# Kuuro-neko/HAI719-Raytracing

Measured on AMD Instinct MI355X. Metric: Msamples/s (pixels x spp / s), Cornell+mesh 1080p@256spp, higher is better.
Workload: dtype f32

## Files before the change

hai719-raytracing_amd/csrc/hrt_api.hip:

```cpp
#include "hrt_kernels.hip"
#include "hrt_dual.hip"
#include "hrt_stream.hip"
#include "hrt_output.hip"
#include "hrt_kat.hip"
#include "hrt_pack.h"

#include <dlfcn.h>
#include <rccl/rccl.h>

#include <array>
#include <cfloat>
#include <chrono>
#include <cmath>
#include <cstdio>
#include <cstdlib>
#include <cstddef>
#include <cstring>
#include <new>
#include <string>
#include <thread>
#include <unordered_map>
#include <vector>

namespace {
// ... 449 lines not shown
}

static int fill_render(hrt_scene *s, const hrt_camera *cam, uint32_t w, uint32_t h, uint32_t spp, uint64_t seed,
                       uint32_t flags, uint32_t rank, uint32_t world, DRender &R, DCamera &C) {
    const int frc = check_frame("render", w, h, k_max_pixels);
    if (frc != HRT_OK) return frc;
    if (!spp) return fail(HRT_ERR_INVALID, "render: spp must be positive");
    if (w > 65535u || h > 65535u) return fail(HRT_ERR_INVALID, "render: w and h must be below 65536 (tile origins are packed in 16 + 16 bits)");
    if (!world || rank >= world) return fail(HRT_ERR_INVALID, "render: bad rank/world");
    R.scene = s->d_scene;
    R.lds_units = (flags & HRT_FLAG_NO_LDS_TREE) ? 0u : s->lds_units;
    R.err_abs = margin_scale(s->bound, std::sqrt(cam->eye[0] * cam->eye[0] + cam->eye[1] * cam->eye[1] + cam->eye[2] * cam->eye[2]));
    {
        const int crc = make_camera(cam, C);
        if (crc != HRT_OK) return crc;
    }
    R.w = w; R.h = h; R.spp = spp;
    R.seed_lo = (uint32_t)seed; R.seed_hi = (uint32_t)(seed >> 32);
    R.flags = flags;
    R.rank = rank; R.world = world;
    R.tiles_x = (w + HRT_TILE - 1) / HRT_TILE;
    R.tiles_total = hrt_tiles_total(w, h);
    R.tiles_owned = hrt_tiles_owned(w, h, rank, world);
    R.tile_counter = s->tile_counter;
    R.stamps = s->stamps;
    R.tile_list = nullptr;
    return HRT_OK;
}

static int size_stream(hrt_scene *s, const KernelBuild &b, DRender &R, uint32_t &grid, uint32_t &lds_bytes) {
    const uint32_t fixed = (uint32_t)(HRT_SP_NQ * HRT_SP_POOL * 2 + HRT_SP_STREAMS * sizeof(SpCtl) + sizeof(SpShared) + HRT_SP_UNITS * sizeof(SpUnit) + HRT_SP_UNITS * HRT_SP_MAXG * 4) +
                           ((b.bits & KB_VIEWS) ? HRT_SP_UNITS * HRT_SP_MAXG * 16u : 0u) +
                           2048u + s->d.tab_rows * 16u
#ifdef HRT_WALK_SEG
                           + 2048u
#endif
                           ;
    uint32_t per_cu = (64u * 4u * HRT_SP_MINW) / HRT_SP_WG;
    while (per_cu > 1u && 160u * 1024u / per_cu < fixed + 16u * 1024u) --per_cu;
    const uint32_t room = (160u * 1024u / per_cu - fixed) / 16u;
    if (!(R.flags & HRT_FLAG_NO_LDS_TREE)) R.lds_units = std::min<uint32_t>(s->d.n_kd_units, room) & ~3u;
    lds_bytes = fixed + R.lds_units * 16u;
    grid = std::min<uint32_t>((uint32_t)g_rt.cus * per_cu, R.tiles_owned);
    {
        const uint32_t per_tile = 64u * std::min<uint32_t>(R.spp, HRT_SP_SCHUNK);
        uint32_t glog = 0;
        while ((2u << glog) <= HRT_SP_MAXG && (per_tile << (glog + 1u)) <= HRT_SP_UNIT) ++glog;
        R.sp_group_log2 = glog;
        uint32_t band = 0;
        while (glog == 0u && band < 2u && ((uint64_t)R.tiles_owned << band) < 64ull * grid && (64u >> (band + 1u)) * (uint64_t)std::min<uint32_t>(R.spp, HRT_SP_SCHUNK) >= 4096u) ++band;
        R.sp_band_log2 = band;
    }
    int rc = s->sp_scratch.grow((size_t)grid * HRT_SP_UNITS * HRT_SP_UNIT * 3u * sizeof(float));
    if (rc == HRT_OK) rc = s->sp_pool.grow((size_t)grid * SP_FIELDS * HRT_SP_POOL * sizeof(uint32_t));
    if (rc != HRT_OK) return rc;
    R.sp_scratch = s->sp_scratch.as<float>();
    R.sp_pool = s->sp_pool.as<uint32_t>();
    return HRT_OK;
}

static int size_lanes(const KernelBuild &b, DRender &R, uint32_t &grid, uint32_t &lds_bytes) {
    const bool dual = b.family == KF_DUAL;
    lds_bytes = R.lds_units * 16u;
    if (dual) {
        const uint32_t wgs = 1024u / HRT_WG, backup = HRT_DS_FIELDS * HRT_WG * 4u;
        const uint32_t room = (156u * 1024u / wgs - backup) / 16u;
        if (R.lds_units > room) R.lds_units = room & ~3u;
        lds_bytes = R.lds_units * 16u + backup;
    }
    int per_cu = 0;
    HIP_TRY(hipOccupancyMaxActiveBlocksPerMultiprocessor(&per_cu, (const void *)b.fn, HRT_WG, lds_bytes));
    if (per_cu < 1) per_cu = 1;
    grid = (uint32_t)(per_cu * g_rt.cus);
    const uint32_t per_wg = (HRT_WG / 64u) * (dual ? 2u : 1u);
    const uint32_t need = (R.tiles_owned + per_wg - 1u) / per_wg;
    if (grid > need) grid = need;
    R.sp_scratch = nullptr;
    R.sp_pool = nullptr;
    return HRT_OK;
}

struct TraceJob {
    uint32_t w, h, s0, spp;
    uint64_t seed;
    uint32_t flags;
    float *d_tiles;
    void *stream;
    uint32_t rank = 0, world = 1;
    bool accumulate = false;
    const uint32_t *list = nullptr;
    uint32_t list_n = 0;
    uint32_t n_views = 0;
};
static int launch_trace(hrt_scene *s, const hrt_camera *cam, const TraceJob &J) {
    DRender R;
    DCamera C;
    int rc = fill_render(s, cam, J.w, J.h, J.spp, J.seed, J.flags, J.rank, J.world, R, C);
    if (rc != HRT_OK) return rc;
    if (J.list) {
        if (J.list_n > R.tiles_owned) return fail(HRT_ERR_INVALID, "render: tile list longer than the rank's tiles");
        R.tile_list = J.list;
        R.tiles_owned = J.list_n;
    }
    if (J.n_views) {
        R.views = s->vw_blocks.as<DView>();
        R.tiles_owned = J.n_views * R.tiles_total;
    }
// ... 378 lines not shown
```

hai719-raytracing_amd/csrc/hrt_stream.hip:

```cpp
#include "hrt_device.h"

#ifndef HRT_SP_POOL
#define HRT_SP_POOL 4096
#endif
#ifndef HRT_SP_WG
#define HRT_SP_WG 1024
#endif
#ifndef HRT_SP_MINW
#define HRT_SP_MINW 4
#endif
#define HRT_SP_SCHUNK 1024
#ifndef HRT_SP_UNIT
#define HRT_SP_UNIT 8192
#endif
#ifndef HRT_SP_UNITS
#define HRT_SP_UNITS 4
#endif
#define HRT_SP_MAXG 16
#ifndef HRT_SP_TRIPS
#define HRT_SP_TRIPS 6
#endif
#ifndef HRT_SP_TPRIO
#define HRT_SP_TPRIO 3
#endif
#ifndef HRT_SP_VOTE
#define HRT_SP_VOTE 0
#endif
#ifndef HRT_SP_STEPS
#define HRT_SP_STEPS 16
#endif
#ifndef HRT_SP_CYCLE_BOUND
#define HRT_SP_CYCLE_BOUND (1u << 16)
#endif
#ifndef HRT_SP_WAIT_SECONDS
#define HRT_SP_WAIT_SECONDS 900ull
#endif
#ifndef HRT_SP_GIVEUP_AFTER
#define HRT_SP_GIVEUP_AFTER 0u
#endif
#ifndef HRT_SP_STREAMS
#define HRT_SP_STREAMS 2
#endif
#ifndef HRT_SP_PMQ
#define HRT_SP_PMQ 1
#endif
#ifndef HRT_SP_THALF
#define HRT_SP_THALF 0
#endif
#ifndef HRT_SP_DEFER
#define HRT_SP_DEFER 1
#endif
#ifndef HRT_SP_PRUNE
#define HRT_SP_PRUNE 3
#endif
#define HRT_SP_QCAP (HRT_SP_POOL / HRT_SP_STREAMS)
#define HRT_SP_NQ 8

namespace hrtk {

enum { SP_OX = 0, SP_OY, SP_OZ, SP_DX, SP_DY, SP_DZ, SP_HT, SP_HID,
       SP_TR, SP_TG, SP_TB, SP_RR, SP_RG, SP_RB, SP_RI, SP_REM,
       SP_WTRI, SP_WTE, SP_WKK, SP_WBT, SP_WREF, SP_WBU, SP_WBV, SP_PM,
       SP_FREE = 24,
       SP_FIELDS = 32 };

struct SpCtl {
    uint32_t cQ[6][2];
    uint32_t cursor;
    uint32_t ngen, gen_n0;
    uint32_t gen_slot, gen_s0;
    uint32_t red_slot;
    uint32_t red_j, red_s0, red_ns;
    uint32_t more;
    uint32_t done, parity;
    uint32_t arrive;
    uint32_t ready;
    uint32_t pad[2];
};
struct SpUnit {
    uint32_t state;
    uint32_t j;
    uint32_t s0, ns;
    uint32_t gen_next, gen_total;
    uint32_t outstanding;
    uint32_t pad;
};
enum { SP_U_FREE = 0, SP_U_READY, SP_U_GENERATING, SP_U_DRAINING, SP_U_REDUCING };
struct SpShared {
    uint32_t lock;
    uint32_t cur;
    uint32_t tiles_done;
    uint32_t abort;
    uint32_t stall;
    uint32_t sections;
    uint32_t pad[2];
};
static_assert(sizeof(SpCtl) % 16 == 0 && sizeof(SpShared) % 16 == 0 && sizeof(SpUnit) % 16 == 0, "the LDS regions behind the control blocks must stay 16-byte aligned");
static_assert(HRT_SP_STREAMS == 1 || HRT_SP_STREAMS == 2, "one or two streams");
static_assert(HRT_SP_UNITS >= 1 && HRT_SP_UNITS <= 4, "a path number carries its unit slot in its two top bits");
static_assert(!HRT_SP_PMQ || HRT_SP_POOL <= 4096, "a T-queue entry is 12 bits of slot id + 4 bits of meshes");
static_assert(HRT_SP_UNIT <= 8192, "g3.w keeps 13 bits of the path's number in its unit beside the bounces left");
static_assert(HRT_SP_QCAP >= 512, "deferring partial chunks needs a queue that can hold a whole chunk whenever fewer than 64 slots are free (6 queues x 63 < QCAP - 64)");

static_assert((HRT_SP_POOL & (HRT_SP_POOL - 1)) == 0 && HRT_SP_POOL <= 65536, "slot ids are 16-bit and masked with HRT_SP_POOL - 1");
static_assert(HRT_SP_NQ * HRT_SP_POOL * 2 + HRT_SP_MAXG * 8 + 512 <= 160 * 1024, "the queues do not fit the CU's 160 KB of LDS");

struct SpLds {
    uint32_t *st;
    uint16_t *q;
    SpCtl *ctl;
};

#define SP_AT(field, slot) ((slot) * (uint32_t)SP_FIELDS + (uint32_t)(field))
__device__ __forceinline__ uint4 sp_ld4(const SpLds &L, int g, uint32_t slot) {
    const v4u v = ((gu4)(L.st + SP_AT(4 * g, slot)))[0];
    return make_uint4(v.x, v.y, v.z, v.w);
}
__device__ __forceinline__ void sp_st4(const SpLds &L, int g, uint32_t slot, uint4 v) {
    v4u w;
    w.x = v.x; w.y = v.y; w.z = v.z; w.w = v.w;
    *((v4u __attribute__((address_space(1))) *)(L.st + SP_AT(4 * g, slot))) = w;
}
#define SP_PIN1(g) "+v"(g.x), "+v"(g.y), "+v"(g.z), "+v"(g.w)
__device__ __forceinline__ uint32_t sp_w7(uint32_t left, uint32_t pnum) { return left | ((pnum & 0x1FFFu) << 3) | (pnum & 0xC0000000u); }
__device__ __forceinline__ uint32_t sp_w7_left(uint32_t w) { return w & 7u; }
__device__ __forceinline__ uint32_t sp_w7_pnum(uint32_t w) { return ((w >> 3) & 0x1FFFu) | (w & 0xC0000000u); }
static_assert(HRT_MAX_SOUP_SLOTS == (1u << 25), "the hit word keeps 25 bits of soup slot");
__device__ __forceinline__ uint32_t sp_hit_word(const Hit &h) {
    return h.kind == 3u ? (3u << 30) | (h.index << 25) | h.tri : (h.kind << 30) | h.index;
}
__device__ __forceinline__ void sp_hit_unword(uint32_t w, Hit &h) {
    h.kind = w >> 30;
    const bool mesh = h.kind == 3u;
    h.index = mesh ? (w >> 25) & 31u : w & 0x3FFFFFFFu;
    h.tri = mesh ? w & 0x01FFFFFFu : 0u;
}
__device__ __forceinline__ uint4 sp_pack(float a, float b, float c, float d) { return make_uint4(__float_as_uint(a), __float_as_uint(b), __float_as_uint(c), __float_as_uint(d)); }
__device__ __forceinline__ void sp_unpack_ray_hit(const uint4 g0, const uint4 g1, Ray &ray, Hit &h) {
    ray.o = mk(__uint_as_float(g0.x), __uint_as_float(g0.y), __uint_as_float(g0.z));
    ray.d = mk(__uint_as_float(g0.w), __uint_as_float(g1.x), __uint_as_float(g1.y));
    h.t = __uint_as_float(g1.z);
    sp_hit_unword(g1.w, h);
    h.a0 = 0.f; h.a1 = 0.f;
}
__device__ __forceinline__ uint4 sp_g1(const Ray &ray, const Hit &h) {
    return make_uint4(__float_as_uint(ray.d.y), __float_as_uint(ray.d.z), __float_as_uint(h.t), sp_hit_word(h));
}
__device__ __forceinline__ void sp_store_ray_hit(const SpLds &L, uint32_t slot, const Ray &ray, const Hit &h) {
    sp_st4(L, 0, slot, sp_pack(ray.o.x, ray.o.y, ray.o.z, ray.d.x));
    sp_st4(L, 1, slot, sp_g1(ray, h));
}
template <class CX>
__device__ __forceinline__ void sp_hit_uv_square(const CX &cx, const Ray &ray, Hit &h) {
    float t, u = 0.f, v = 0.f;
    if (quad_t(cx.tq + HRT_QUAD_ROWS * h.index, ray, HRT_FLT_MAX, t, u, v)) { h.a0 = u; h.a1 = v; }
}
template <class CX>
__device__ __forceinline__ void sp_hit_uv_triangle(const CX &cx, const Ray &ray, Hit &h) {
    const gf4 tr = (gf4)cx.S->tris + HRT_TRI_ROWS * h.tri;
    float u1, u2;
    (void)tri_inside(ld(tr, 0), ld(tr, 1), ld(tr, 2), ray, h.t, u1, u2);
    h.a0 = u1; h.a1 = u2;
}
__device__ __forceinline__ uint16_t *spq(const SpLds &L, int which, uint32_t parity) { return L.q + (2 * which + parity) * HRT_SP_QCAP; }

#define SP_TO_NONE 6u
__device__ __forceinline__ void sp_push_all(const SpLds &L, SpCtl &C, uint32_t out, uint32_t to, uint32_t slot) {
    uint32_t rank = 0, count = 0, leader = 0;
#pragma unroll
    for (uint32_t q = 0; q < 6u; ++q) {
        const uint64_t m = __ballot(to == q);
        if (to == q) {
            rank = __builtin_amdgcn_mbcnt_hi((uint32_t)(m >> 32), __builtin_amdgcn_mbcnt_lo((uint32_t)m, 0u));
            count = (uint32_t)__popcll(m);
            leader = (uint32_t)__builtin_ctzll(m | (1ull << 63));
        }
    }
    uint32_t base = 0;
    if (to < SP_TO_NONE && rank == 0u) base = atomicAdd(&C.cQ[to][out], count);
    base = __shfl(base, (int)leader);
    if (to < SP_TO_NONE) {
        const uint32_t pos = base + rank;
        const uint32_t buf = to == 0u ? 0u : (to == 5u ? 3u : ((to == 2u || to == 3u) ? 1u : 2u));
        const bool back = to == 3u || to == 4u;
        spq(L, (int)buf, out)[back ? (uint32_t)HRT_SP_QCAP - 1u - pos : pos] = (uint16_t)slot;
    }
}

template <bool LIGHTS, bool EXACT = false, bool SPHF = false, bool LIST = false, bool VIEWS = false>
__device__ __forceinline__ void stream_body(const DRender &R) {
    extern __shared__ uint4 s_raw[];
    SpLds L;
    L.st = R.sp_pool + (size_t)blockIdx.x * ((size_t)SP_FIELDS * HRT_SP_POOL);
    L.q = reinterpret_cast<uint16_t *>(s_raw);
    L.ctl = reinterpret_cast<SpCtl *>(L.q + HRT_SP_NQ * HRT_SP_POOL);
    SpShared &SH = *reinterpret_cast<SpShared *>(L.ctl + HRT_SP_STREAMS);
    SpUnit *const U = reinterpret_cast<SpUnit *>(&SH + 1);
    uint32_t *tile_xy = reinterpret_cast<uint32_t *>(U + HRT_SP_UNITS);
    uint4 *tile_vw = reinterpret_cast<uint4 *>(tile_xy + HRT_SP_UNITS * HRT_SP_MAXG);
    float *s_lut = VIEWS ? reinterpret_cast<float *>(tile_vw + HRT_SP_UNITS * HRT_SP_MAXG)
                         : reinterpret_cast<float *>(tile_xy + HRT_SP_UNITS * HRT_SP_MAXG);
    float4 *s_tabs = reinterpret_cast<float4 *>(s_lut + 512);
    CtxT<EXACT, true, SPHF> cx;
    cx.S = (cscene)R.scene;
    const uint32_t tab_rows = cx.S->tab_rows;
    uint4 *s_units = reinterpret_cast<uint4 *>(s_tabs + tab_rows);
    cx.set_tables((lf4)s_tabs, (lf1)s_lut, cx.S);
    cx.lds = (lu4)s_units;
    cx.lds_n = R.lds_units;
    cx.err_abs = R.err_abs;
    cx.flags = R.flags;
    unsigned long long stamps_local[17];
    cx.st = stamps_local;
#ifdef HRT_WALK_SEG
    {
        unsigned long long *wseg = reinterpret_cast<unsigned long long *>(s_units + R.lds_units) + (threadIdx.x >> 6) * 16u;
        if ((threadIdx.x & 63u) < 16u) wseg[threadIdx.x & 63u] = 0ull;
        cx.st = wseg;
    }
#endif
    ccam cam = (ccam)R.cam;
    const uint32_t tid = threadIdx.x, lane = tid & 63u;
    {
        gu4 g_units = (gu4)cx.S->kd_units;
        for (uint32_t i = tid; i < cx.lds_n; i += HRT_SP_WG) s_units[i] = ld(g_units, i);
        gf4 g_tabs = (gf4)cx.S->tabs;
        for (uint32_t i = tid; i < tab_rows; i += HRT_SP_WG) s_tabs[i] = ld(g_tabs, i);
        if (tid < 512u) s_lut[tid] = c_u8_lut[tid];
    }
    uint16_t *const q_all = L.q;
    if (tid < HRT_SP_STREAMS) {
        SpCtl &C0 = L.ctl[tid];
        C0.cQ[0][0] = C0.cQ[0][1] = 0;
        for (int k = 0; k < 4; ++k) C0.cQ[1 + k][0] = C0.cQ[1 + k][1] = 0;
        C0.cQ[5][0] = HRT_SP_QCAP; C0.cQ[5][1] = 0;
        C0.parity = 1; C0.done = 0; C0.arrive = 0; C0.ready = 0; C0.cursor = 0; C0.ngen = 0; C0.gen_n0 = 0; C0.gen_slot = 0; C0.gen_s0 = 0;
        C0.red_slot = HRT_SP_UNITS; C0.red_j = 0; C0.red_s0 = 0; C0.red_ns = 0; C0.more = 1;
        if (tid == 0) {
            SH.lock = 0; SH.cur = 0; SH.tiles_done = 0; SH.abort = 0; SH.stall = 0; SH.sections = 0;
            for (int k = 0; k < HRT_SP_UNITS; ++k) { U[k].state = SP_U_FREE; U[k].j = 0; U[k].s0 = 0; U[k].ns = 0; U[k].gen_next = 0; U[k].gen_total = 0; U[k].outstanding = 0; }
        }
    }
    for (uint32_t i = tid; i < HRT_SP_POOL; i += HRT_SP_WG)
        q_all[(i / HRT_SP_QCAP) * (HRT_SP_NQ * HRT_SP_QCAP) + (2 * 3 + 0) * HRT_SP_QCAP + (i % HRT_SP_QCAP)] = (uint16_t)i;
    const bool has_mesh = cx.S->n_meshes != 0u;
    const bool multi_mesh = cx.S->n_meshes > 1u;
#if HRT_SP_PMQ
    const bool pm_in_entry = cx.S->n_meshes <= 4u;
#endif
    const bool prune = !EXACT && HRT_SP_PRUNE != 0 && cx.S->prune_ok != 0u;
    const bool moving = cx.S->any_motion != 0u;
    const bool sky_is_zero = cx.S->skybox_image < 0 && cx.S->dark_sky != 0;
    float *scratch = R.sp_scratch + (size_t)blockIdx.x * ((size_t)HRT_SP_UNITS * HRT_SP_UNIT * 3u);
    const uint32_t glog = R.sp_group_log2, G = 1u << glog, blog = R.sp_band_log2;
    const uint32_t upix = (64u << glog) >> blog, upix_log2 = 6u + glog - blog;
    const uint32_t items = R.tiles_owned << blog;
    auto view_row = [&](uint32_t pnum) { return tile_vw[(pnum >> 30) * HRT_SP_MAXG + (((pnum & 0x3FFFFFFFu) & (upix - 1u)) >> 6)]; };
#define SP_UNI(x) __builtin_amdgcn_readfirstlane(x)

#ifndef HRT_SP_SEG_KIND
#define HRT_SP_SEG_KIND 1
#endif
#ifdef HRT_SP_SEG
    unsigned long long seg[10] = {0, 0, 0, 0, 0, 0, 0, 0, 0, 0}, seg_last = 0;
    bool seg_on = false;
#define SEG_START(on) do { seg_on = (on); if (seg_on) { asm volatile("s_waitcnt vmcnt(0) lgkmcnt(0)" ::: "memory"); seg_last = __builtin_readcyclecounter(); } } while (0)
#define SEG(k) do { if (seg_on) { asm volatile("s_waitcnt vmcnt(0) lgkmcnt(0)" ::: "memory"); const unsigned long long t_ = __builtin_readcyclecounter(); \
                                  seg[k] += t_ - seg_last; seg_last = t_; } } while (0)
#else
#define SEG_START(on) do { } while (0)
#define SEG(k) do { } while (0)
#endif
#ifdef HRT_SP_DEBUG
    unsigned long long dbg_work = 0, dbg_chunks = 0, dbg_cycles = 0, dbg_serial = 0, dbg_wait = 0, dbg_drain = 0, dbg_tail = 0, dbg_tail_cycles = 0;
    unsigned long long dbg_class[6] = {0, 0, 0, 0, 0, 0};
    const unsigned long long dbg_t0 = __builtin_readcyclecounter();
#endif
    const uint32_t per_fold = min((uint32_t)HRT_SP_SCHUNK, (uint32_t)HRT_SP_UNIT / upix);
    auto serial_section = [&](SpCtl &C, uint16_t *qs) {
        const uint32_t par = SP_UNI(C.parity) ^ 1u;
        const uint32_t free_in = SP_UNI(C.cQ[5][par]);
#if HRT_SP_DEFER
        const uint32_t want = free_in & ~63u;
#else
        const uint32_t want = free_in;
#endif
        if (lane == 0) {
            uint32_t spins = 0;
            while (atomicCAS(&SH.lock, 0u, 1u) != 0u) {
                __builtin_amdgcn_s_sleep(1);
// ... 61 lines not shown
                    atomicAdd(&u.outstanding, ngen);
                    if (u.gen_next == u.gen_total) u.state = SP_U_DRAINING;
                    gs = cur;
                }
            }
            bool generating = false, idle = SH.tiles_done != 0u;
            for (uint32_t k = 0; k < HRT_SP_UNITS; ++k) {
                generating = generating || U[k].state == SP_U_READY || U[k].state == SP_U_GENERATING || (U[k].state == SP_U_FREE && SH.tiles_done == 0u);
                idle = idle && U[k].state == SP_U_FREE;
            }
            C.ngen = ngen; C.gen_n0 = n0; C.gen_slot = gs; C.gen_s0 = U[gs].s0;
            C.more = generating ? 1u : 0u;
            C.done = idle ? 1u : 0u;
            uint32_t entries = ngen + (red < HRT_SP_UNITS ? 1u : 0u);
            for (int q = 0; q < 5; ++q) entries += (HRT_SP_DEFER && generating) ? (C.cQ[q][par] & ~63u) : C.cQ[q][par];
            const uint32_t stalled = entries != 0u ? (SH.stall = 0u) : ++SH.stall;
            const uint32_t sections = ++SH.sections;
            if (stalled > HRT_SP_CYCLE_BOUND || (HRT_SP_GIVEUP_AFTER != 0u && sections > HRT_SP_GIVEUP_AFTER)) {
                if (R.stamps) {
                    __hip_atomic_store(R.stamps + 15, 0xDEADull, __ATOMIC_RELAXED, __HIP_MEMORY_SCOPE_SYSTEM);
                    R.stamps[14] = 2;
                    for (uint32_t k = 0; k < HRT_SP_UNITS; ++k) R.stamps[8 + k] = ((unsigned long long)U[k].state << 48) | ((unsigned long long)U[k].outstanding << 24) | U[k].gen_next;
                    R.stamps[12] = ((unsigned long long)SH.tiles_done << 32) | SH.cur; R.stamps[13] = ((unsigned long long)want << 32) | C.cQ[0][par];
                }
                __hip_atomic_store(&SH.abort, 1u, __ATOMIC_RELAXED, __HIP_MEMORY_SCOPE_WORKGROUP);
            }
            __hip_atomic_store(&SH.lock, 0u, __ATOMIC_RELEASE, __HIP_MEMORY_SCOPE_WORKGROUP);
        }
        asm volatile("s_waitcnt lgkmcnt(0)" ::: "memory");
        const uint32_t ngen = SP_UNI(C.ngen);
        uint16_t *qFi = qs + (2 * 3 + par) * HRT_SP_QCAP, *qFo = qs + (2 * 3 + (par ^ 1u)) * HRT_SP_QCAP;
        for (uint32_t i = lane; i < free_in - ngen; i += 64u) qFo[i] = qFi[ngen + i];
        const bool defer = HRT_SP_DEFER && SP_UNI(C.more) != 0u;
        const uint32_t cT = SP_UNI(C.cQ[0][par]), rT = defer ? (cT & 63u) : 0u;
        if (lane < rT) qs[(2 * 0 + (par ^ 1u)) * HRT_SP_QCAP + lane] = qs[(2 * 0 + par) * HRT_SP_QCAP + cT - rT + lane];
        uint32_t cKv[4], rK[4], waiting = cT;
#pragma unroll
        for (int k = 0; k < 4; ++k) {
            cKv[k] = SP_UNI(C.cQ[1 + k][par]);
            rK[k] = defer ? (cKv[k] & 63u) : 0u;
            waiting += cKv[k];
            const int which = (k == 1 || k == 2) ? 1 : 2;
            const bool back = !(k == 1 || k == 0);
            const uint16_t *qi = qs + (2 * which + par) * HRT_SP_QCAP;
            uint16_t *qo = qs + (2 * which + (par ^ 1u)) * HRT_SP_QCAP;
            if (lane < rK[k]) {
                const uint32_t e = cKv[k] - rK[k] + lane;
                qo[back ? (uint32_t)HRT_SP_QCAP - 1u - lane : lane] = qi[back ? (uint32_t)HRT_SP_QCAP - 1u - e : e];
            }
        }
        if (lane == 0) {
#pragma unroll
            for (int k = 0; k < 4; ++k) { C.cQ[1 + k][par] = cKv[k] - rK[k]; C.cQ[1 + k][par ^ 1u] = rK[k]; }
            C.cQ[0][par] = cT - rT;
            C.cQ[0][par ^ 1u] = rT;
            C.cQ[5][par ^ 1u] = free_in - ngen;
            C.cursor = 0; C.parity = par;
            C.done = (C.done != 0u && ngen == 0u && waiting == 0u && C.red_slot == HRT_SP_UNITS) ? 1u : 0u;
        }
        asm volatile("s_waitcnt lgkmcnt(0)" ::: "memory");
        if (lane == 0) __hip_atomic_store(&C.ready, C.ready + 1u, __ATOMIC_RELEASE, __HIP_MEMORY_SCOPE_WORKGROUP);
    };
    __syncthreads();
    if (tid < 64u)
        for (uint32_t st = 0; st < HRT_SP_STREAMS; ++st) serial_section(L.ctl[st], q_all + st * (HRT_SP_NQ * HRT_SP_QCAP));
    __syncthreads();
    uint32_t fin[HRT_SP_UNITS];
    for (int k = 0; k < HRT_SP_UNITS; ++k) fin[k] = 0u;

    uint32_t kcyc[HRT_SP_STREAMS], fin_mask = 0u;
    for (uint32_t st = 0; st < HRT_SP_STREAMS; ++st) kcyc[st] = 1u;
    for (uint32_t round = 0;; ++round) {
        const uint32_t st = HRT_SP_STREAMS == 1 ? 0u : (round & 1u);
        if (fin_mask == (1u << HRT_SP_STREAMS) - 1u) break;
        if (fin_mask & (1u << st)) continue;
        SpCtl &C = L.ctl[st];
        L.q = q_all + st * (HRT_SP_NQ * HRT_SP_QCAP);
        {
#ifdef HRT_SP_DEBUG
            const unsigned long long dbg_q0 = __builtin_readcyclecounter();
#endif
            uint32_t spins = 0, aborted = 0;
            const unsigned long long wait_t0 = __builtin_amdgcn_s_memrealtime();
            while (SP_UNI(__hip_atomic_load(&C.ready, __ATOMIC_ACQUIRE, __HIP_MEMORY_SCOPE_WORKGROUP)) < kcyc[st]) {
                __builtin_amdgcn_s_sleep(8);
                aborted = SP_UNI(__hip_atomic_load(&SH.abort, __ATOMIC_RELAXED, __HIP_MEMORY_SCOPE_WORKGROUP));
                if (aborted) break;
                if ((++spins & 1023u) == 0u && (spins >> 10) > 16u && __builtin_amdgcn_s_memrealtime() - wait_t0 > 100000000ull * HRT_SP_WAIT_SECONDS) {
                    if (lane == 0) {
                        if (R.stamps) { __hip_atomic_store(R.stamps + 15, 0xDEADull, __ATOMIC_RELAXED, __HIP_MEMORY_SCOPE_SYSTEM); R.stamps[14] = 3; }
                        __hip_atomic_store(&SH.abort, 1u, __ATOMIC_RELAXED, __HIP_MEMORY_SCOPE_WORKGROUP);
                    }
                    aborted = 1u;
                    break;
                }
            }
#ifdef HRT_SP_DEBUG
            dbg_wait += __builtin_readcyclecounter() - dbg_q0;
#endif
            if (aborted || SP_UNI(__hip_atomic_load(&SH.abort, __ATOMIC_RELAXED, __HIP_MEMORY_SCOPE_WORKGROUP))) break;
        }
        if (SP_UNI(C.done)) { fin_mask |= 1u << st; continue; }
        const uint32_t parity = SP_UNI(C.parity);
        const uint32_t ngen = SP_UNI(C.ngen), n0 = SP_UNI(C.gen_n0), gs = SP_UNI(C.gen_slot), s0 = SP_UNI(C.gen_s0);
        const uint32_t red = SP_UNI(C.red_slot), nR = red < HRT_SP_UNITS ? (upix * 3u + 63u) >> 6 : 0u;
        const uint32_t cTin = SP_UNI(C.cQ[0][parity]);
        const uint32_t cK0 = SP_UNI(C.cQ[1][parity]), cK1 = SP_UNI(C.cQ[2][parity]), cK2 = SP_UNI(C.cQ[3][parity]),
                       cK3 = SP_UNI(C.cQ[4][parity]);
        const uint32_t nT = HRT_SP_THALF ? (cTin + 31u) >> 5 : (cTin + 63u) >> 6, e3 = nT + ((cK3 + 63u) >> 6), e1 = e3 + ((cK1 + 63u) >> 6),
                       e2 = e1 + ((cK2 + 63u) >> 6), e0 = e2 + ((cK0 + 63u) >> 6), nG = (ngen + 63u) >> 6, total = e0 + nG;
        uint16_t *qTi = spq(L, 0, parity);
        uint16_t *qAi = spq(L, 1, parity), *qBi = spq(L, 2, parity);
        uint16_t *qFi = spq(L, 3, parity);
#ifdef HRT_SP_DEBUG
        const unsigned long long dbg_w0 = __builtin_readcyclecounter();
        ++dbg_cycles;
#endif

        for (;;) {
            uint32_t c = 0;
            if (lane == 0) c = atomicAdd(&C.cursor, 1u);
            c = SP_UNI(c);
            if (c >= nR + total) break;
            if (c < nR) {
                const uint32_t i = c * 64u + lane;
                const uint32_t rj = SP_UNI(C.red_j), rs0 = SP_UNI(C.red_s0), rns = SP_UNI(C.red_ns);
                if (i < upix * 3u && rj + i / (192u >> blog) < items) {
                    float *out = R.out_tiles + (size_t)rj * (192u >> blog) + i;
                    float acc = (rs0 != 0u || R.accumulate) ? *out : 0.f;
                    const float *col = scratch + (size_t)red * ((size_t)HRT_SP_UNIT * 3u) + i;
                    const uint32_t stride = upix * 3u;
                    uint32_t sm = 0;
                    for (; sm + 8u <= rns; sm += 8u) {
                        float v[8];
#pragma unroll
                        for (int k = 0; k < 8; ++k) v[k] = col[(size_t)(sm + k) * stride];
#pragma unroll
                        for (int k = 0; k < 8; ++k) acc += v[k];
                    }
                    for (; sm < rns; ++sm) acc += col[(size_t)sm * stride];
                    if (rs0 + rns >= R.spp) {
                        const uint32_t q = i / 3u, p = q & 63u, txy = tile_xy[red * HRT_SP_MAXG + (q >> 6)];
                        const uint32_t px = (txy & 0xFFFFu) + (p & 7u), py = (txy >> 16) + (p >> 3);
                        if (!(px < R.w && py < R.h)) acc = 0.f;
                        else if (!R.accumulate) acc = acc / (float)R.spp;
                    }
                    *out = acc;
                }
                continue;
            }
            c -= nR;
#ifdef HRT_SP_DEBUG
            ++dbg_chunks;
            const unsigned long long dbg_c0 = __builtin_readcyclecounter();
            const uint32_t dbg_k = c < nT ? 0u : (c < e3 ? 1u : (c < e1 ? 2u : (c < e2 ? 3u : (c < e0 ? 4u : 5u))));
#endif
            if (c < nT) {
#if HRT_SP_TPRIO
                __builtin_amdgcn_s_setprio(HRT_SP_TPRIO);
#endif
                const uint32_t e = HRT_SP_THALF ? c * 32u + lane : c * 64u + lane;
                const bool act = e < cTin && (!HRT_SP_THALF || lane < 32u);
                uint32_t slot = 0, kind = 0, pm = 0, t_before = 0;
                bool walked = false;
                Ray ray;
                ray.o = mk(0.f, 0.f, 0.f); ray.d = mk(0.f, 0.f, 1.f); ray.time = 0.f;
                Hit h;
                h.kind = 0; h.index = 0; h.t = HRT_FLT_MAX; h.tri = 0; h.a0 = 0.f; h.a1 = 0.f;
                Walk w;
                w.ref = HRT_KD_NIL; w.t_entry = 0.f; w.kk = 0xFFFFu; w.best_t = HRT_FLT_MAX; w.best_tri = 0; w.bu = 0.f; w.bv = 0.f;
                SEG_START(HRT_SP_SEG_KIND == 2);
                if (act) {
#if HRT_SP_PMQ
                    const uint32_t entry = qTi[e];
                    slot = entry & (HRT_SP_POOL - 1u);
#else
                    slot = qTi[e] & (HRT_SP_POOL - 1u);
#endif
                    uint4 g0 = sp_ld4(L, 0, slot), g1 = sp_ld4(L, 1, slot), g4 = sp_ld4(L, 4, slot), g5 = sp_ld4(L, 5, slot);
                    asm volatile("" : SP_PIN1(g0), SP_PIN1(g1), SP_PIN1(g4), SP_PIN1(g5));
                    sp_unpack_ray_hit(g0, g1, ray, h);
                    pm = g5.w;
                    t_before = g1.z;
                    w.ref = g5.x; w.t_entry = __uint_as_float(g4.y); w.kk = g4.z; w.best_t = __uint_as_float(g4.w);
                    w.best_tri = g4.x; w.bu = __uint_as_float(g5.y); w.bv = __uint_as_float(g5.z);
#if HRT_SP_PMQ
                    if (pm_in_entry && (entry >> 12) != 0u) { w.ref = HRT_KD_NIL; pm = entry >> 12; }
#endif
                }
#ifdef HRT_SP_SEG
                asm volatile("" : "+v"(ray.o.x), "+v"(w.t_entry), "+v"(h.t));
#endif
                SEG(0);
                if (act) {
#if HRT_SP_VOTE
                    walked = walk_vote(cx, ray, pm, w, h, HRT_SP_STEPS);
#else
                    walked = multi_mesh ? walk_some_per_lane(cx, ray, pm, w, h, HRT_SP_TRIPS) : walk_some(cx, ray, pm, w, h, HRT_SP_TRIPS);
#endif
                }
                SEG(1);
                if (act) {
                    if (__float_as_uint(h.t) != t_before) sp_st4(L, 1, slot, sp_g1(ray, h));
                    if (!walked) {
                        sp_st4(L, 4, slot, make_uint4(w.best_tri, __float_as_uint(w.t_entry), w.kk, __float_as_uint(w.best_t)));
                        sp_st4(L, 5, slot, make_uint4(w.ref, __float_as_uint(w.bu), __float_as_uint(w.bv), pm));
                    }
                    kind = h.kind;
                }
#if HRT_SP_TPRIO
                __builtin_amdgcn_s_setprio(0);
#endif
                sp_push_all(L, C, parity ^ 1u, !act ? SP_TO_NONE : (walked ? 1u + kind : 0u), slot);
                SEG(2);
#ifdef HRT_SP_SEG
                if (seg_on) { seg[7] += 1; seg[6] += (unsigned long long)__popcll(__ballot(act)); seg[5] += (unsigned long long)__popcll(__ballot(act && walked)); }
#endif
            } else {
                const bool is_gen = c >= e0;
                const uint32_t first = is_gen ? e0 : (c < e3 ? nT : (c < e1 ? e3 : (c < e2 ? e1 : e2)));
                const uint32_t fill = is_gen ? ngen : (c < e3 ? cK3 : (c < e1 ? cK1 : (c < e2 ? cK2 : cK0)));
                const bool from_back = !is_gen && (c < e3 || (c >= e1 && c < e2));
                const uint16_t *qHi = (c < e3 || c >= e2) ? qBi : qAi;
                const uint32_t e = (c - first) * 64u + lane;
                const bool act = e < fill;
                uint32_t slot = 0, kind = 0, fin_unit = 0, pnum = 0;
                bool trace = false, freed = false;
                bool ended = false, last_seg = false;
                f3 rad = mk(0.f, 0.f, 0.f);
                SEG_START((HRT_SP_SEG_KIND == 1 && !is_gen && c >= e1 && c < e2) || (HRT_SP_SEG_KIND == 3 && !is_gen && c >= e3 && c < e1) ||
                          (HRT_SP_SEG_KIND == 4 && is_gen) || (HRT_SP_SEG_KIND == 5 && !is_gen && c < e3));
                Ray ray;
                ray.o = mk(0.f, 0.f, 0.f); ray.d = mk(0.f, 0.f, 1.f); ray.time = 0.f;
                if (act && is_gen) {
                    slot = qFi[e] & (HRT_SP_POOL - 1u);
                    const uint32_t n = n0 + e;
                    const uint32_t q = n & (upix - 1u), s = s0 + (n >> upix_log2);
                    const uint32_t p = q & 63u, txy = tile_xy[gs * HRT_SP_MAXG + (q >> 6)];
                    const uint32_t px = (txy & 0xFFFFu) + (p & 7u), py = (txy >> 16) + (p >> 3);
                    if (txy != 0xFFFFFFFFu && px < R.w && py < R.h) {
                        uint4 vw = make_uint4(0u, R.seed_lo, R.seed_hi, 0u);
                        if (VIEWS) { vw = view_row(n | (gs << 30)); cx.err_abs = __uint_as_float(vw.w); }
                        Rng rng;
                        rng.start(vw.y, vw.z, py * R.w + px, R.s0 + s);
                        const float u = ((float)px + rng.next()) / (float)R.w;
                        const float v = ((float)py + rng.next()) / (float)R.h;
                        const float tm = rng.next();
                        if (VIEWS) {
                            for (uint64_t todo = __ballot(1); todo != 0ull;) {
                                const uint32_t view = __builtin_amdgcn_readlane(vw.x, __builtin_ctzll(todo));
                                const bool mine = vw.x == view;
                                if (mine) ray = camera_ray<EXACT>((ccam)&((cview)R.views + view)->cam, u, v, tm);
                                todo &= ~__ballot(mine);
                            }
                        } else {
                            ray = camera_ray<EXACT>(cam, u, v, tm);
                        }
                        pnum = n | (gs << 30);
                        sp_st4(L, 2, slot, sp_pack(1.f, 1.f, 1.f, 0.f));
                        sp_st4(L, 3, slot, make_uint4(0u, 0u, rng.i, sp_w7(6u, pnum)));
                        trace = true;
                    } else {
                        float *o = scratch + (size_t)gs * ((size_t)HRT_SP_UNIT * 3u) + (size_t)n * 3u;
                        o[0] = 0.f; o[1] = 0.f; o[2] = 0.f;
                        freed = true;
                        fin_unit = gs;
                    }
                } else if (act) {
                    slot = qHi[from_back ? (uint32_t)HRT_SP_QCAP - 1u - e : e] & (HRT_SP_POOL - 1u);
                    uint4 g0 = sp_ld4(L, 0, slot), g1 = sp_ld4(L, 1, slot), g2 = sp_ld4(L, 2, slot), g3 = sp_ld4(L, 3, slot);
                    asm volatile("" : SP_PIN1(g0), SP_PIN1(g1), SP_PIN1(g2), SP_PIN1(g3));
                    pnum = sp_w7_pnum(g3.w);
                    Rng key;
                    {
                        const uint32_t kn = pnum & 0x3FFFFFFFu, ku = pnum >> 30;
                        const uint32_t kq = kn & (upix - 1u), ks = U[ku].s0 + (kn >> upix_log2);
                        const uint32_t kxy = tile_xy[ku * HRT_SP_MAXG + (kq >> 6)];
                        const uint32_t kx = (kxy & 0xFFFFu) + (kq & 7u), ky = (kxy >> 16) + ((kq & 63u) >> 3);
                        uint4 vw = make_uint4(0u, R.seed_lo, R.seed_hi, 0u);
                        if (VIEWS) { vw = view_row(pnum); cx.err_abs = __uint_as_float(vw.w); }
                        key.start(vw.y, vw.z, ky * R.w + kx, R.s0 + ks);
                        key.i = 2u;
                    }
                    Hit h;
                    sp_unpack_ray_hit(g0, g1, ray, h);
                    ray.time = moving ? key.next() : 0.f;
                    f3 thr = mk(__uint_as_float(g2.x), __uint_as_float(g2.y), __uint_as_float(g2.z));
                    rad = mk(__uint_as_float(g2.w), __uint_as_float(g3.x), __uint_as_float(g3.y));
                    int remaining = (int)sp_w7_left(g3.w);
#ifdef HRT_SP_SEG
                    asm volatile("" : "+v"(remaining), "+v"(ray.o.x), "+v"(thr.x), "+v"(rad.x));
#endif
                    SEG(0);
                    if (h.kind == 0u) {
                        rad = rad + thr * sky(cx, ray.d, remaining);
                        ended = true;
                    } else {
                        Rng rng;
                        rng.k0 = key.k0; rng.k1 = key.k1; rng.i = g3.z;
                        if (h.kind == 2u) sp_hit_uv_square(cx, ray, h);
                        else if (h.kind == 3u) sp_hit_uv_triangle(cx, ray, h);
                        const Surface sf = shade(cx, ray, h);
                        SEG(1);
                        f3 direct = mk(0.f, 0.f, 0.f);
                        if (LIGHTS) direct = direct_light(cx, sf, ray, rng);
                        SEG(8);
                        rad = rad + thr * (direct + sf.emission);
                        thr = thr * sf.albedo;
                        scatter(sf, ray, rng);
                        SEG(2);
                        --remaining;
                        ended = (remaining == 0);
                        if ((HRT_SP_PRUNE & 1) && prune && thr.x == 0.f && thr.y == 0.f && thr.z == 0.f) ended = true;
                        if (!ended) {
                            sp_st4(L, 2, slot, sp_pack(thr.x, thr.y, thr.z, rad.x));
                            sp_st4(L, 3, slot, make_uint4(__float_as_uint(rad.y), __float_as_uint(rad.z), rng.i, sp_w7((uint32_t)remaining, pnum)));
                            trace = true;
                            last_seg = (HRT_SP_PRUNE & 2) && !LIGHTS && prune && remaining == 1;
                        }
                    }
                }
                bool to_mesh = false;
                SEG(3);
                Hit hn;
                hn.kind = 0; hn.index = 0; hn.t = HRT_FLT_MAX; hn.tri = 0; hn.a0 = 0.f; hn.a1 = 0.f;
                uint32_t pmn = 0;
                if (trace) {
                    hn = prims_hit(cx, ray);
                    SEG(4);
                    pmn = has_mesh ? mesh_gates(cx, ray) : 0u;
                    SEG(5);
                }
                if (SPHF && trace && hn.kind == 0u && pmn == 0u) {
                    f3 thr = mk(1.f, 1.f, 1.f);
                    int remaining = 6;
                    if (!is_gen) {
                        const uint4 g2 = sp_ld4(L, 2, slot), g3 = sp_ld4(L, 3, slot);
                        thr = mk(__uint_as_float(g2.x), __uint_as_float(g2.y), __uint_as_float(g2.z));
                        rad = mk(__uint_as_float(g2.w), __uint_as_float(g3.x), __uint_as_float(g3.y));
                        remaining = (int)sp_w7_left(g3.w);
                    }
                    rad = rad + thr * sky(cx, ray.d, remaining);
                    trace = false; ended = true; last_seg = false;
                }
                if (last_seg) {
                    bool dead;
                    if (hn.kind == 0u) {
                        dead = sky_is_zero;
                    } else {
                        const uint32_t mat = hn.kind == 1u ? __float_as_uint(ld(cx.ts, HRT_SPHERE_ROWS * hn.index + 1u).w)
                                                           : __float_as_uint(ld(cx.tq, HRT_QUAD_ROWS * hn.index + 4u).w);
                        dead = __float_as_uint(ld(cx.tm, HRT_MAT_ROWS * mat + 1u).w) == 0u;
                    }
                    if (dead) { trace = false; ended = true; }
                }
                if (ended) {
                    const uint32_t n = min(pnum & 0x3FFFFFFFu, (uint32_t)HRT_SP_UNIT - 1u);
                    fin_unit = pnum >> 30;
                    float *o = scratch + (size_t)fin_unit * ((size_t)HRT_SP_UNIT * 3u) + (size_t)n * 3u;
                    o[0] = rad.x / 6.f; o[1] = rad.y / 6.f; o[2] = rad.z / 6.f;
                    freed = true;
                }
                if (trace) {
                    sp_store_ray_hit(L, slot, ray, hn);
#if HRT_SP_PMQ
                    if (!pm_in_entry)
#endif
                    if (pmn != 0u) sp_st4(L, 5, slot, make_uint4(HRT_KD_NIL, 0u, 0u, pmn));
                    to_mesh = pmn != 0u;
                    kind = hn.kind;
                }
#if HRT_SP_PMQ
                sp_push_all(L, C, parity ^ 1u, trace ? (to_mesh ? 0u : 1u + kind) : (freed ? 5u : SP_TO_NONE), (trace && to_mesh && pm_in_entry) ? (slot | (pmn << 12)) : slot);
#else
                sp_push_all(L, C, parity ^ 1u, trace ? (to_mesh ? 0u : 1u + kind) : (freed ? 5u : SP_TO_NONE), slot);
#endif
#pragma unroll
                for (uint32_t k = 0; k < HRT_SP_UNITS; ++k) fin[k] += (uint32_t)__popcll(__ballot(freed && fin_unit == k));
                SEG(6);
#ifdef HRT_SP_SEG
                if (seg_on) seg[7] += 1;
#endif
            }
#ifdef HRT_SP_DEBUG
            dbg_class[dbg_k] += __builtin_readcyclecounter() - dbg_c0;
#endif
        }
#ifdef HRT_SP_DEBUG
        dbg_work += __builtin_readcyclecounter() - dbg_w0;
        if (ngen == 0u) { dbg_tail += __builtin_readcyclecounter() - dbg_w0; ++dbg_tail_cycles; }
#endif
        asm volatile("s_waitcnt vmcnt(0) lgkmcnt(0)" ::: "memory");
        if (lane == 0) {
#pragma unroll
            for (uint32_t k = 0; k < HRT_SP_UNITS; ++k)
                if (fin[k]) atomicSub(&U[k].outstanding, fin[k]);
        }
#pragma unroll
        for (uint32_t k = 0; k < HRT_SP_UNITS; ++k) fin[k] = 0u;
        uint32_t arrived = 0;
        if (lane == 0) arrived = __hip_atomic_fetch_add(&C.arrive, 1u, __ATOMIC_ACQ_REL, __HIP_MEMORY_SCOPE_WORKGROUP);
        arrived = SP_UNI(arrived);
#ifdef HRT_SP_DEBUG
        const unsigned long long dbg_s0 = __builtin_readcyclecounter();
#endif
        if (arrived + 1u == (HRT_SP_WG / 64u) * kcyc[st]) serial_section(C, L.q);
#ifdef HRT_SP_DEBUG
        dbg_serial += __builtin_readcyclecounter() - dbg_s0;
#endif
        ++kcyc[st];
    }
    L.q = q_all;
    __syncthreads();
    if (SP_UNI(__hip_atomic_load(&SH.abort, __ATOMIC_RELAXED, __HIP_MEMORY_SCOPE_WORKGROUP))) return;

#ifdef HRT_SP_SEG
    if (lane == 0 && R.stamps)
        for (int k = 0; k < 9; ++k) atomicAdd(R.stamps + k, seg[k]);
#endif
#ifdef HRT_WALK_SEG
    if (lane == 0 && R.stamps)
        for (int k = 0; k < 12; ++k) atomicAdd(R.stamps + k, cx.st[k]);
#endif
#ifdef HRT_SP_DEBUG
    if (lane == 0 && R.stamps) {
        atomicAdd(R.stamps + 0, dbg_work); atomicAdd(R.stamps + 1, __builtin_readcyclecounter() - dbg_t0);
        atomicAdd(R.stamps + 2, dbg_cycles); atomicAdd(R.stamps + 3, dbg_chunks); atomicAdd(R.stamps + 4, dbg_serial);
        for (int k = 0; k < 6; ++k) atomicAdd(R.stamps + 5 + k, dbg_class[k]);
        atomicAdd(R.stamps + 11, dbg_wait); atomicAdd(R.stamps + 12, dbg_drain); atomicAdd(R.stamps + 13, dbg_tail); atomicAdd(R.stamps + 14, dbg_tail_cycles);
// ... 24 lines not shown
```

Before: 3856.

## Store hit-queue path records positionally in SoA blocks beside queue entries

Path state for rays headed to the sphere/quad hit queues is now written into a per-queue-position record array laid out as 64-entry structure-of-arrays blocks, so consecutive lanes in a chunk read and write contiguous memory instead of scattering through slot-indexed records. Queue entries carry a positional flag bit, the ray/hit and throughput/radiance records are written once after the push instead of in separate places, and an extra tail-copy work item relocates partial-chunk remainders between parity buffers. This aims to cut uncoalesced global traffic for the stream pool, at the cost of more scratch memory, extra copy work for tails, and more complex indexing.

```diff
diff --git a/hai719-raytracing_amd/csrc/hrt_api.hip b/hai719-raytracing_amd/csrc/hrt_api.hip
--- a/hai719-raytracing_amd/csrc/hrt_api.hip
+++ b/hai719-raytracing_amd/csrc/hrt_api.hip
@@ -525,7 +525,7 @@
         R.sp_band_log2 = band;
     }
     int rc = s->sp_scratch.grow((size_t)grid * HRT_SP_UNITS * HRT_SP_UNIT * 3u * sizeof(float));
-    if (rc == HRT_OK) rc = s->sp_pool.grow((size_t)grid * SP_FIELDS * HRT_SP_POOL * sizeof(uint32_t));
+    if (rc == HRT_OK) rc = s->sp_pool.grow((size_t)grid * SP_WG_DWORDS * sizeof(uint32_t));
     if (rc != HRT_OK) return rc;
     R.sp_scratch = s->sp_scratch.as<float>();
     R.sp_pool = s->sp_pool.as<uint32_t>();
diff --git a/hai719-raytracing_amd/csrc/hrt_stream.hip b/hai719-raytracing_amd/csrc/hrt_stream.hip
--- a/hai719-raytracing_amd/csrc/hrt_stream.hip
+++ b/hai719-raytracing_amd/csrc/hrt_stream.hip
@@ -75,7 +75,8 @@
     uint32_t done, parity;
     uint32_t arrive;
     uint32_t ready;
-    uint32_t pad[2];
+    uint32_t tails;
+    uint32_t pad;
 };
 struct SpUnit {
     uint32_t state;
@@ -104,9 +105,12 @@
 
 static_assert((HRT_SP_POOL & (HRT_SP_POOL - 1)) == 0 && HRT_SP_POOL <= 65536, "slot ids are 16-bit and masked with HRT_SP_POOL - 1");
 static_assert(HRT_SP_NQ * HRT_SP_POOL * 2 + HRT_SP_MAXG * 8 + 512 <= 160 * 1024, "the queues do not fit the CU's 160 KB of LDS");
+static_assert(HRT_SP_POOL <= 32768, "a hit-queue entry keeps SP_POSITIONAL in bit 15, above the slot id");
+static_assert(HRT_SP_QCAP % 64 == 0, "a chunk's 64 queue positions are one block of the hit-record array, from either end");
 
 struct SpLds {
     uint32_t *st;
+    uint32_t hr;
     uint16_t *q;
     SpCtl *ctl;
 };
@@ -122,6 +126,29 @@
     *((v4u __attribute__((address_space(1))) *)(L.st + SP_AT(4 * g, slot))) = w;
 }
 #define SP_PIN1(g) "+v"(g.x), "+v"(g.y), "+v"(g.z), "+v"(g.w)
+#define SP_POSITIONAL 0x8000u
+#define SP_HR_STREAM (2u * 2u * (uint32_t)HRT_SP_QCAP * 16u)
+#define SP_HR_WG ((uint32_t)HRT_SP_STREAMS * SP_HR_STREAM)
+#define SP_WG_DWORDS ((uint32_t)SP_FIELDS * HRT_SP_POOL + SP_HR_WG)
+__device__ __forceinline__ uint32_t sp_hr_at(uint32_t buf, uint32_t parity, uint32_t idx) {
+    return ((parity * 2u + (buf - 1u)) * (uint32_t)HRT_SP_QCAP + (idx & ~63u)) * 16u + (idx & 63u) * 4u;
+}
+struct SpRec { uint32_t at, gs; };
+__device__ __forceinline__ SpRec sp_rec(const SpLds &L, bool positional, uint32_t slot, uint32_t buf, uint32_t parity, uint32_t idx) {
+    SpRec r;
+    r.at = positional ? L.hr + sp_hr_at(buf, parity, idx) : SP_AT(0, slot);
+    r.gs = positional ? 256u : 4u;
+    return r;
+}
+__device__ __forceinline__ uint4 sp_ld4(const SpLds &L, const SpRec &r, uint32_t g) {
+    const v4u v = ((gu4)(L.st + (r.at + g * r.gs)))[0];
+    return make_uint4(v.x, v.y, v.z, v.w);
+}
+__device__ __forceinline__ void sp_st4(const SpLds &L, const SpRec &r, uint32_t g, uint4 v) {
+    v4u w;
+    w.x = v.x; w.y = v.y; w.z = v.z; w.w = v.w;
+    *((v4u __attribute__((address_space(1))) *)(L.st + (r.at + g * r.gs))) = w;
+}
 __device__ __forceinline__ uint32_t sp_w7(uint32_t left, uint32_t pnum) { return left | ((pnum & 0x1FFFu) << 3) | (pnum & 0xC0000000u); }
 __device__ __forceinline__ uint32_t sp_w7_left(uint32_t w) { return w & 7u; }
 __device__ __forceinline__ uint32_t sp_w7_pnum(uint32_t w) { return ((w >> 3) & 0x1FFFu) | (w & 0xC0000000u); }
@@ -146,10 +173,6 @@
 __device__ __forceinline__ uint4 sp_g1(const Ray &ray, const Hit &h) {
     return make_uint4(__float_as_uint(ray.d.y), __float_as_uint(ray.d.z), __float_as_uint(h.t), sp_hit_word(h));
 }
-__device__ __forceinline__ void sp_store_ray_hit(const SpLds &L, uint32_t slot, const Ray &ray, const Hit &h) {
-    sp_st4(L, 0, slot, sp_pack(ray.o.x, ray.o.y, ray.o.z, ray.d.x));
-    sp_st4(L, 1, slot, sp_g1(ray, h));
-}
 template <class CX>
 __device__ __forceinline__ void sp_hit_uv_square(const CX &cx, const Ray &ray, Hit &h) {
     float t, u = 0.f, v = 0.f;
@@ -165,7 +188,7 @@
 __device__ __forceinline__ uint16_t *spq(const SpLds &L, int which, uint32_t parity) { return L.q + (2 * which + parity) * HRT_SP_QCAP; }
 
 #define SP_TO_NONE 6u
-__device__ __forceinline__ void sp_push_all(const SpLds &L, SpCtl &C, uint32_t out, uint32_t to, uint32_t slot) {
+__device__ __forceinline__ uint32_t sp_push_all(const SpLds &L, SpCtl &C, uint32_t out, uint32_t to, uint32_t slot) {
     uint32_t rank = 0, count = 0, leader = 0;
 #pragma unroll
     for (uint32_t q = 0; q < 6u; ++q) {
@@ -179,19 +202,23 @@
     uint32_t base = 0;
     if (to < SP_TO_NONE && rank == 0u) base = atomicAdd(&C.cQ[to][out], count);
     base = __shfl(base, (int)leader);
+    uint32_t idx = 0;
     if (to < SP_TO_NONE) {
         const uint32_t pos = base + rank;
         const uint32_t buf = to == 0u ? 0u : (to == 5u ? 3u : ((to == 2u || to == 3u) ? 1u : 2u));
         const bool back = to == 3u || to == 4u;
-        spq(L, (int)buf, out)[back ? (uint32_t)HRT_SP_QCAP - 1u - pos : pos] = (uint16_t)slot;
+        idx = back ? (uint32_t)HRT_SP_QCAP - 1u - pos : pos;
+        spq(L, (int)buf, out)[idx] = (uint16_t)slot;
     }
+    return idx;
 }
 
 template <bool LIGHTS, bool EXACT = false, bool SPHF = false, bool LIST = false, bool VIEWS = false>
 __device__ __forceinline__ void stream_body(const DRender &R) {
     extern __shared__ uint4 s_raw[];
     SpLds L;
-    L.st = R.sp_pool + (size_t)blockIdx.x * ((size_t)SP_FIELDS * HRT_SP_POOL);
+    L.st = R.sp_pool + (size_t)blockIdx.x * (size_t)SP_WG_DWORDS;
+    L.hr = (uint32_t)SP_FIELDS * HRT_SP_POOL;
     L.q = reinterpret_cast<uint16_t *>(s_raw);
     L.ctl = reinterpret_cast<SpCtl *>(L.q + HRT_SP_NQ * HRT_SP_POOL);
     SpShared &SH = *reinterpret_cast<SpShared *>(L.ctl + HRT_SP_STREAMS);
@@ -235,7 +262,7 @@
         for (int k = 0; k < 4; ++k) C0.cQ[1 + k][0] = C0.cQ[1 + k][1] = 0;
         C0.cQ[5][0] = HRT_SP_QCAP; C0.cQ[5][1] = 0;
         C0.parity = 1; C0.done = 0; C0.arrive = 0; C0.ready = 0; C0.cursor = 0; C0.ngen = 0; C0.gen_n0 = 0; C0.gen_slot = 0; C0.gen_s0 = 0;
-        C0.red_slot = HRT_SP_UNITS; C0.red_j = 0; C0.red_s0 = 0; C0.red_ns = 0; C0.more = 1;
+        C0.red_slot = HRT_SP_UNITS; C0.red_j = 0; C0.red_s0 = 0; C0.red_ns = 0; C0.more = 1; C0.tails = 0;
         if (tid == 0) {
             SH.lock = 0; SH.cur = 0; SH.tiles_done = 0; SH.abort = 0; SH.stall = 0; SH.sections = 0;
             for (int k = 0; k < HRT_SP_UNITS; ++k) { U[k].state = SP_U_FREE; U[k].j = 0; U[k].s0 = 0; U[k].ns = 0; U[k].gen_next = 0; U[k].gen_total = 0; U[k].outstanding = 0; }
@@ -403,6 +430,7 @@
         if (lane == 0) {
 #pragma unroll
             for (int k = 0; k < 4; ++k) { C.cQ[1 + k][par] = cKv[k] - rK[k]; C.cQ[1 + k][par ^ 1u] = rK[k]; }
+            C.tails = rK[0] | (rK[1] << 6) | (rK[2] << 12) | (rK[3] << 18);
             C.cQ[0][par] = cT - rT;
             C.cQ[0][par ^ 1u] = rT;
             C.cQ[5][par ^ 1u] = free_in - ngen;
@@ -427,6 +455,7 @@
         if (fin_mask & (1u << st)) continue;
         SpCtl &C = L.ctl[st];
         L.q = q_all + st * (HRT_SP_NQ * HRT_SP_QCAP);
+        L.hr = (uint32_t)SP_FIELDS * HRT_SP_POOL + st * SP_HR_STREAM;
         {
 #ifdef HRT_SP_DEBUG
             const unsigned long long dbg_q0 = __builtin_readcyclecounter();
@@ -455,6 +484,7 @@
         const uint32_t parity = SP_UNI(C.parity);
         const uint32_t ngen = SP_UNI(C.ngen), n0 = SP_UNI(C.gen_n0), gs = SP_UNI(C.gen_slot), s0 = SP_UNI(C.gen_s0);
         const uint32_t red = SP_UNI(C.red_slot), nR = red < HRT_SP_UNITS ? (upix * 3u + 63u) >> 6 : 0u;
+        const uint32_t nRC = nR + (SP_UNI(C.tails) != 0u ? 4u : 0u);
         const uint32_t cTin = SP_UNI(C.cQ[0][parity]);
         const uint32_t cK0 = SP_UNI(C.cQ[1][parity]), cK1 = SP_UNI(C.cQ[2][parity]), cK2 = SP_UNI(C.cQ[3][parity]),
                        cK3 = SP_UNI(C.cQ[4][parity]);
@@ -472,7 +502,7 @@
             uint32_t c = 0;
             if (lane == 0) c = atomicAdd(&C.cursor, 1u);
             c = SP_UNI(c);
-            if (c >= nR + total) break;
+            if (c >= nRC + total) break;
             if (c < nR) {
                 const uint32_t i = c * 64u + lane;
                 const uint32_t rj = SP_UNI(C.red_j), rs0 = SP_UNI(C.red_s0), rns = SP_UNI(C.red_ns);
@@ -500,7 +530,24 @@
                 }
                 continue;
             }
-            c -= nR;
+            if (c < nRC) {
+                const uint32_t k = c - nR, r = (SP_UNI(C.tails) >> (6u * k)) & 63u;
+                const uint32_t base = k == 0u ? cK0 : (k == 1u ? cK1 : (k == 2u ? cK2 : cK3));
+                const uint32_t buf = (k == 1u || k == 2u) ? 1u : 2u;
+                const bool back = k >= 2u;
+                if (lane < r) {
+                    const uint32_t from = back ? (uint32_t)HRT_SP_QCAP - 1u - (base + lane) : base + lane;
+                    const uint32_t to = back ? (uint32_t)HRT_SP_QCAP - 1u - lane : lane;
+                    if (spq(L, (int)buf, parity ^ 1u)[to] & SP_POSITIONAL) {
+                        const SpRec ri = sp_rec(L, true, 0u, buf, parity, from), ro = sp_rec(L, true, 0u, buf, parity ^ 1u, to);
+                        uint4 g0 = sp_ld4(L, ri, 0), g1 = sp_ld4(L, ri, 1), g2 = sp_ld4(L, ri, 2), g3 = sp_ld4(L, ri, 3);
+                        asm volatile("" : SP_PIN1(g0), SP_PIN1(g1), SP_PIN1(g2), SP_PIN1(g3));
+                        sp_st4(L, ro, 0, g0); sp_st4(L, ro, 1, g1); sp_st4(L, ro, 2, g2); sp_st4(L, ro, 3, g3);
+                    }
+                }
+                continue;
+            }
+            c -= nRC;
 #ifdef HRT_SP_DEBUG
             ++dbg_chunks;
             const unsigned long long dbg_c0 = __builtin_readcyclecounter();
@@ -578,7 +625,9 @@
                 uint32_t slot = 0, kind = 0, fin_unit = 0, pnum = 0;
                 bool trace = false, freed = false;
                 bool ended = false, last_seg = false;
-                f3 rad = mk(0.f, 0.f, 0.f);
+                f3 rad = mk(0.f, 0.f, 0.f), thr = mk(1.f, 1.f, 1.f);
+                uint32_t rng_i = 0;
+                int remaining = 6;
                 SEG_START((HRT_SP_SEG_KIND == 1 && !is_gen && c >= e1 && c < e2) || (HRT_SP_SEG_KIND == 3 && !is_gen && c >= e3 && c < e1) ||
                           (HRT_SP_SEG_KIND == 4 && is_gen) || (HRT_SP_SEG_KIND == 5 && !is_gen && c < e3));
                 Ray ray;
@@ -608,8 +657,7 @@
                             ray = camera_ray<EXACT>(cam, u, v, tm);
                         }
                         pnum = n | (gs << 30);
-                        sp_st4(L, 2, slot, sp_pack(1.f, 1.f, 1.f, 0.f));
-                        sp_st4(L, 3, slot, make_uint4(0u, 0u, rng.i, sp_w7(6u, pnum)));
+                        rng_i = rng.i;
                         trace = true;
                     } else {
                         float *o = scratch + (size_t)gs * ((size_t)HRT_SP_UNIT * 3u) + (size_t)n * 3u;
@@ -618,8 +666,10 @@
                         fin_unit = gs;
                     }
                 } else if (act) {
-                    slot = qHi[from_back ? (uint32_t)HRT_SP_QCAP - 1u - e : e] & (HRT_SP_POOL - 1u);
-                    uint4 g0 = sp_ld4(L, 0, slot), g1 = sp_ld4(L, 1, slot), g2 = sp_ld4(L, 2, slot), g3 = sp_ld4(L, 3, slot);
+                    const uint32_t qi = from_back ? (uint32_t)HRT_SP_QCAP - 1u - e : e, entry = qHi[qi];
+                    slot = entry & (HRT_SP_POOL - 1u);
+                    const SpRec rec = sp_rec(L, (entry & SP_POSITIONAL) != 0u, slot, (c < e3 || c >= e2) ? 2u : 1u, parity, qi);
+                    uint4 g0 = sp_ld4(L, rec, 0), g1 = sp_ld4(L, rec, 1), g2 = sp_ld4(L, rec, 2), g3 = sp_ld4(L, rec, 3);
                     asm volatile("" : SP_PIN1(g0), SP_PIN1(g1), SP_PIN1(g2), SP_PIN1(g3));
                     pnum = sp_w7_pnum(g3.w);
                     Rng key;
@@ -636,9 +686,9 @@
                     Hit h;
                     sp_unpack_ray_hit(g0, g1, ray, h);
                     ray.time = moving ? key.next() : 0.f;
-                    f3 thr = mk(__uint_as_float(g2.x), __uint_as_float(g2.y), __uint_as_float(g2.z));
+                    thr = mk(__uint_as_float(g2.x), __uint_as_float(g2.y), __uint_as_float(g2.z));
                     rad = mk(__uint_as_float(g2.w), __uint_as_float(g3.x), __uint_as_float(g3.y));
-                    int remaining = (int)sp_w7_left(g3.w);
+                    remaining = (int)sp_w7_left(g3.w);
 #ifdef HRT_SP_SEG
                     asm volatile("" : "+v"(remaining), "+v"(ray.o.x), "+v"(thr.x), "+v"(rad.x));
 #endif
@@ -664,8 +714,7 @@
                         ended = (remaining == 0);
                         if ((HRT_SP_PRUNE & 1) && prune && thr.x == 0.f && thr.y == 0.f && thr.z == 0.f) ended = true;
                         if (!ended) {
-                            sp_st4(L, 2, slot, sp_pack(thr.x, thr.y, thr.z, rad.x));
-                            sp_st4(L, 3, slot, make_uint4(__float_as_uint(rad.y), __float_as_uint(rad.z), rng.i, sp_w7((uint32_t)remaining, pnum)));
+                            rng_i = rng.i;
                             trace = true;
                             last_seg = (HRT_SP_PRUNE & 2) && !LIGHTS && prune && remaining == 1;
                         }
@@ -683,14 +732,6 @@
                     SEG(5);
                 }
                 if (SPHF && trace && hn.kind == 0u && pmn == 0u) {
-                    f3 thr = mk(1.f, 1.f, 1.f);
-                    int remaining = 6;
-                    if (!is_gen) {
-                        const uint4 g2 = sp_ld4(L, 2, slot), g3 = sp_ld4(L, 3, slot);
-                        thr = mk(__uint_as_float(g2.x), __uint_as_float(g2.y), __uint_as_float(g2.z));
-                        rad = mk(__uint_as_float(g2.w), __uint_as_float(g3.x), __uint_as_float(g3.y));
-                        remaining = (int)sp_w7_left(g3.w);
-                    }
                     rad = rad + thr * sky(cx, ray.d, remaining);
                     trace = false; ended = true; last_seg = false;
                 }
@@ -713,19 +754,27 @@
                     freed = true;
                 }
                 if (trace) {
-                    sp_store_ray_hit(L, slot, ray, hn);
+                    to_mesh = pmn != 0u;
+                    kind = hn.kind;
+                }
+                const uint32_t to = trace ? (to_mesh ? 0u : 1u + kind) : (freed ? 5u : SP_TO_NONE);
+                uint32_t entry = slot;
+                if (trace && !to_mesh) entry = slot | SP_POSITIONAL;
+#if HRT_SP_PMQ
+                if (trace && to_mesh && pm_in_entry) entry = slot | (pmn << 12);
+#endif
+                const uint32_t at = sp_push_all(L, C, parity ^ 1u, to, entry);
+                if (trace) {
+                    const SpRec rec = sp_rec(L, !to_mesh, slot, (to == 2u || to == 3u) ? 1u : 2u, parity ^ 1u, at);
+                    sp_st4(L, rec, 0, sp_pack(ray.o.x, ray.o.y, ray.o.z, ray.d.x));
+                    sp_st4(L, rec, 1, sp_g1(ray, hn));
+                    sp_st4(L, rec, 2, sp_pack(thr.x, thr.y, thr.z, rad.x));
+                    sp_st4(L, rec, 3, make_uint4(__float_as_uint(rad.y), __float_as_uint(rad.z), rng_i, sp_w7((uint32_t)remaining, pnum)));
 #if HRT_SP_PMQ
                     if (!pm_in_entry)
 #endif
                     if (pmn != 0u) sp_st4(L, 5, slot, make_uint4(HRT_KD_NIL, 0u, 0u, pmn));
-                    to_mesh = pmn != 0u;
-                    kind = hn.kind;
-                }
-#if HRT_SP_PMQ
-                sp_push_all(L, C, parity ^ 1u, trace ? (to_mesh ? 0u : 1u + kind) : (freed ? 5u : SP_TO_NONE), (trace && to_mesh && pm_in_entry) ? (slot | (pmn << 12)) : slot);
-#else
-                sp_push_all(L, C, parity ^ 1u, trace ? (to_mesh ? 0u : 1u + kind) : (freed ? 5u : SP_TO_NONE), slot);
-#endif
+                }
 #pragma unroll
                 for (uint32_t k = 0; k < HRT_SP_UNITS; ++k) fin[k] += (uint32_t)__popcll(__ballot(freed && fin_unit == k));
                 SEG(6);
```

Result: faster. 4006, median of 6 (+3.9%).
